# alenxav/bWGR

Measured on AMD Instinct MI355X. Metric: MCMC iter/sec (full marker sweep), higher is better.
Workload: dtype f32 scalars, fixed-point / f64 residual, int8 genotypes; 1 GPU; c4: synthetic n=10000 x p=1000000 int8, BayesB pi=0.99 (1.2% of the markers in the model at the last sweep), exact chain (blocked sweep, block=128, 40 slabs x 256 rows + 1 sequencer, the chain alone on the GPU: 80 streamers x 128 rows, engine generation 3, lag 12 blocks); n=10000, p=1000000, model=BayesB, df=5, chains=1

## Files before the change

### bwgr_amd/csrc/sweep3.hip.h

```cpp
#pragma once
#include "sweep2.hip.h"

namespace bwgr {

#ifdef BWGR_STAMPS
#define S3ST_DECL unsigned long long ph3[8] = {0, 0, 0, 0, 0, 0, 0, 0}, tl3 = __builtin_amdgcn_s_memtime()
#define S3ST(k, cond) do { if ((BWGR_STAMPS == 1 || (BWGR_STAMPS == 2 && ((k) == 0 || (k) == 1 || (k) == 4)) || (BWGR_STAMPS == 3 && ((k) == 0 || (k) == 4) && blockIdx.x == 0 && threadIdx.x == 0) || (BWGR_STAMPS == 4 && (k) <= 5 && blockIdx.x == 0 && threadIdx.x == 0)) && (cond)) { const unsigned long long t_ = __builtin_amdgcn_s_memtime(); ph3[k] += t_ - tl3; tl3 = t_; } } while (0)
#define S3ST_FLUSH(base, cond) do { if ((cond) && a.stamps) for (int k_ = 0; k_ < 8; ++k_) atomicAdd(&a.stamps[(base) + k_], ph3[k_]); } while (0)
#else
#define S3ST_DECL do { } while (0)
#define S3ST(k, cond) do { } while (0)
#define S3ST_FLUSH(base, cond) do { } while (0)
#endif

static constexpr int S3_MAXD = 16;
static constexpr int S3_LSTRIDE = 2 * SW_MAXM + 2;
static constexpr int S3_ND = 7;
static constexpr int S3_RING = S3_MAXD * SW_MAXM;
static constexpr int S3_GPD_BYTES = 16384;
static constexpr int S3_ROWSLOT = 1024;
static constexpr int S3_NRX = 8;
static constexpr int S3_OS = 12;
static constexpr int S3_NFW = 4;
static constexpr int S3_NFL = 8;
// ... 227 lines not shown
  s += (size_t)2 * S3_NFW * S3_NFL * SW_MAXM * (g16 ? 2 : 4);
  if (g16) s += (size_t)3 * S3_GPD_BYTES + (size_t)S3_NRX * S3_ROWSLOT;
  s += (size_t)3 * S3_QRAW_BYTES;
  return s + 256 + 512;
}

__device__ __forceinline__ void s3_streamer(const Sweep3Args &A) {
#ifdef BWGR_EXPERIMENTS
  const int SDBG = A.dbg;
#else
  constexpr int SDBG = 0;
#endif
  extern __shared__ __attribute__((aligned(16))) unsigned char smem[];
  const SweepArgs &a = A.a;
  const int tid = threadIdx.x, lane = tid & 63, wave = tid >> 6;
  const int m16 = lane & 15, grp = lane >> 4;
  const int w = s3_stream_index(A);
  const unsigned long long *lists_w = A.lists;
  const int m = a.m, R = a.R, R3 = A.R3, Rp = R3 + 16, D = A.D;
  const int slab = w / A.sub, hsub = w - slab * A.sub;
  const int nb = a.blk_end - a.blk_begin;
  const int NU = R3 >> 6;
  const int ND = 8 - NU;
  const int cprs = (R3 == 256) ? 4 : (R3 == 128 ? 3 : 2);
  const int8_t *Xs = reinterpret_cast<const int8_t *>(a.X) + (size_t)slab * a.p * R + (size_t)hsub * R3;
  const int64_t row0 = (int64_t)slab * R + (int64_t)hsub * R3;
  uint32_t *abortw = a.xflags + (size_t)a.K * SW_FLAG_STRIDE;
  const size_t tile_b = (size_t)SW_MAXM * Rp;
  int8_t *tile0 = reinterpret_cast<int8_t *>(smem);
  size_t off = 2 * tile_b;
  int8_t *edig0 = reinterpret_cast<int8_t *>(smem + off); off += (size_t)2 * 16 * Rp;
  int8_t *ddig0 = reinterpret_cast<int8_t *>(smem + off); off += (size_t)2 * 16 * S2_DP;
  int *outu = reinterpret_cast<int *>(smem + off); off += (size_t)64 * S3_OS * 4 * 4;
  int *outd = reinterpret_cast<int *>(smem + off); off += (size_t)8 * 32 * S3_OS * 4;
  uint32_t *ctl_s = reinterpret_cast<uint32_t *>(smem + off);
  const int sh = a.sc->e3_sh;
  const double S = s3_pow2(sh), invS = s3_pow2(-sh);
  auto blk_j0 = [&](int b) { return (a.blk_begin + b) * m; };
  auto blk_m = [&](int b) { return min(m, a.p - (a.blk_begin + b) * m); };

  for (int i = tid; i < (int)((2 * 16 * Rp + 2 * 16 * S2_DP) / 4); i += SW_THREADS) reinterpret_cast<uint32_t *>(edig0)[i] = 0u;
  if (tid < 16) ctl_s[tid] = 0u;
  long long e_own = 0;
  const bool upd = wave < NU;
  if (upd) e_own = __double2ll_rn(a.e[row0 + 64 * wave + lane] * S);

  s3_u4 ta0 = {0, 0, 0, 0}, ta1 = ta0, ta2 = ta0, ta3 = ta0, tb0 = ta0, tb1 = ta0, tb2 = ta0, tb3 = ta0;
#define S3_TILE_EACH(X) X(0, tp0) X(1, tp1) X(2, tp2) X(3, tp3)
#define S3_ISSUE1(u, name) { const int cc_ = min(tid + (u) * SW_THREADS, tot_ - 1); const int jj_ = min(cc_ >> cprs, mBt_ - 1), ii_ = cc_ & ((1 << cprs) - 1); \
    name = __builtin_nontemporal_load(reinterpret_cast<const s3_u4 *>(Xs + (size_t)(j0t_ + jj_) * R + ii_ * 16)); }
#define S3_TILE_ISSUE(b_) do { const int j0t_ = blk_j0(b_), mBt_ = blk_m(b_), tot_ = m << cprs; S3_TILE_EACH(S3_ISSUE1) } while (0)
#define S3_COMMIT1(u, name) { const int c_ = tid + (u) * SW_THREADS; if (c_ < tot_) { const int jj_ = c_ >> cprs, ii_ = c_ & ((1 << cprs) - 1); \
    *reinterpret_cast<s3_u4 *>(dst_ + (size_t)jj_ * Rp + ii_ * 16) = name; } }
#define S3_TILE_COMMIT(b_) do { int8_t *dst_ = tile0 + (size_t)((b_) & 1) * tile_b; const int tot_ = m << cprs; S3_TILE_EACH(S3_COMMIT1) } while (0)

  auto fold_list = [&](int bs, unsigned long long pre) -> int {
    const int Bs = a.blk_begin + bs;
    const unsigned long long *L = lists_w + (size_t)Bs * S3_LSTRIDE;
    const int8_t *col = Xs + (size_t)(Bs * m) * R + 64 * wave + lane;
    const uint64_t t0 = wall_clock64();
    unsigned spins = 0;
    unsigned long long hv = __builtin_amdgcn_readfirstlane((uint32_t)pre) | ((unsigned long long)__builtin_amdgcn_readfirstlane((uint32_t)(pre >> 32)) << 32);
    while (!s3_epoch_is(hv, A.epoch)) {
      hv = ld_agent_raw64(L);
      hv = __builtin_amdgcn_readfirstlane((uint32_t)hv) | ((unsigned long long)__builtin_amdgcn_readfirstlane((uint32_t)(hv >> 32)) << 32);
      if (s3_epoch_is(hv, A.epoch)) break;
      if ((++spins & 63u) == 0u) {
// ... 18 lines not shown
        }
        __builtin_amdgcn_s_sleep(1);
      }
      const uint32_t wlo = (uint32_t)wv, whi = (uint32_t)(wv >> 32);
      for (int e0 = 0; e0 < nw / 2; e0 += 8) {
        int xb[8]; long long cq[8];
#pragma unroll
        for (int u = 0; u < 8; ++u) {
          const int ee = min(e0 + u, nw / 2 - 1);
          const uint32_t a0 = __builtin_amdgcn_readlane(wlo, 1 + 2 * ee), a1 = __builtin_amdgcn_readlane(whi, 1 + 2 * ee);
          const uint32_t b0 = __builtin_amdgcn_readlane(wlo, 2 + 2 * ee);
          const int k = (int)(a1 & 0xFFu);
          cq[u] = (e0 + u < nw / 2) ? (long long)(((unsigned long long)b0 << 32) | (unsigned long long)a0) : 0ll;
          xb[u] = upd ? (int)col[(size_t)k * R] : 0;
        }
#pragma unroll
        for (int u = 0; u < 8; ++u) e_own -= (long long)xb[u] * cq[u];
      }
    }
    return 1;
  };

  {
    s3_u4 &tp0 = ta0, &tp1 = ta1, &tp2 = ta2, &tp3 = ta3;
    S3_TILE_ISSUE(0);
    S3_TILE_COMMIT(0);
    if (nb > 2) S3_TILE_ISSUE(2);
  }
  if (nb > 1) { s3_u4 &tp0 = tb0, &tp1 = tb1, &tp2 = tb2, &tp3 = tb3; S3_TILE_ISSUE(1); }
  float drej_pre = a.ps.blocks[a.blk_begin].drej[tid & (SW_MAXM - 1)];
  unsigned long long lpre = 0ull;
  __syncthreads();
  S3ST_DECL;
  const bool st_u = (w == 0 && tid == 0), st_d = (w == 0 && tid == 64 * NU);

  auto step = [&](int b, s3_u4 &tp0, s3_u4 &tp1, s3_u4 &tp2, s3_u4 &tp3) -> bool {
    const int mB = blk_m(b), par = b & 1;
    S3ST(0, st_u || st_d);
    int8_t *tile = tile0 + (size_t)par * tile_b;
    int8_t *edig = edig0 + (size_t)par * 16 * Rp;
    int8_t *ddig = ddig0 + (size_t)par * 16 * S2_DP;
    if (b >= D && upd && !(SDBG & 512)) { if (!fold_list(b - D, lpre)) ctl_s[0] = 1u; }
    S3ST(1, st_u);
    if (upd) {
      if ((unsigned long long)(e_own + (1ll << 54)) >> 55) ctl_s[1] = 1u;
      s3_put_digits7(e_own, edig + 64 * wave + lane, Rp);
    } else if (tid >= SW_THREADS - SW_MAXM) {
      const double qd = (tid - (SW_THREADS - SW_MAXM) < mB) ? rint((double)drej_pre * S) : 0.0;
      if (!(fabs(qd) < 18014398509481984.0)) ctl_s[1] = 1u;
      s3_put_digits7((long long)qd, ddig + (tid - (SW_THREADS - SW_MAXM)), S2_DP);
    }
    S3ST(2, st_u);
#if defined(BWGR_STAMPS) && BWGR_STAMPS == 2
    S3ST(0, st_u || st_d);
    asm volatile("s_waitcnt lgkmcnt(0)\n\ts_barrier" ::: "memory");
    S3ST(4, st_u || st_d);
#else
    asm volatile("s_waitcnt lgkmcnt(0)\n\ts_barrier" ::: "memory");
    S3ST(3, st_u || st_d);
#endif
    if (ctl_s[0]) { if (tid == 0) a.sc->error = 1u; return false; }
    if (b + 1 < nb) S3_TILE_COMMIT(b + 1);
    S3ST(6, st_u || st_d);
    {
      const int bn1 = min(b + 1, nb - 1);
      drej_pre = a.ps.blocks[a.blk_begin + bn1].drej[tid & (SW_MAXM - 1)];
      lpre = ld_agent_raw64(lists_w + (size_t)(a.blk_begin + max(bn1 - D, 0)) * S3_LSTRIDE + lane);
// ... 84 lines not shown
  if (upd && ((unsigned long long)(e_own + (1ll << 54)) >> 55)) ctl_s[1] = 1u;
  __syncthreads();
  if (ctl_s[0]) { if (tid == 0) a.sc->error = 1u; return; }
  if (ctl_s[1] && tid == 0) a.sc->error = 2u;
  if (upd) a.e[row0 + 64 * wave + lane] = (double)e_own * invS;
#undef S3_TILE_EACH
#undef S3_ISSUE1
#undef S3_TILE_ISSUE
#undef S3_COMMIT1
#undef S3_TILE_COMMIT
}

template <int R3, int NTB>
__device__ __forceinline__ void s3_streamer_dma(const Sweep3Args &A) {
#ifdef BWGR_EXPERIMENTS
  const int SDBG = A.dbg;
#else
  constexpr int SDBG = 0;
#endif
  extern __shared__ __attribute__((aligned(16))) unsigned char smem[];
  const SweepArgs &a = A.a;
  const int tid = threadIdx.x, lane = tid & 63, wave = tid >> 6;
  const int m16 = lane & 15, grp = lane >> 4;
  const int w = s3_stream_index(A);
  const unsigned long long *lists_w = A.lists;
  const int m = a.m, R = a.R, D = A.D;
  constexpr int Rp = R3 + 16;
  constexpr int CH = R3 / 16;
  constexpr int MPP = 1024 / R3;
  constexpr int NPC = SW_MAXM / MPP;
  static_assert(R3 == 128 || R3 == 256, "sixteen or thirty-two pieces");
  const int slab = w / A.sub, hsub = w - slab * A.sub;
  const int nb = a.blk_end - a.blk_begin;
  constexpr int NU = R3 >> 6, ND = 8 - NU;
  const int8_t *Xs = reinterpret_cast<const int8_t *>(a.X) + (size_t)slab * a.p * R + (size_t)hsub * R3;
  const int64_t row0 = (int64_t)slab * R + (int64_t)hsub * R3;
  uint32_t *abortw = a.xflags + (size_t)a.K * SW_FLAG_STRIDE;
  constexpr size_t tile_b = (size_t)SW_MAXM * R3;
  int8_t *tile0 = reinterpret_cast<int8_t *>(smem);
  size_t off = NTB * tile_b;
  const uint32_t tile_la = (uint32_t)__builtin_amdgcn_readfirstlane((int)(uint32_t)(uintptr_t)(__attribute__((address_space(3))) const unsigned char *)smem);
  int8_t *edig0 = reinterpret_cast<int8_t *>(smem + off); off += (size_t)2 * 16 * Rp;
  int8_t *ddig0 = reinterpret_cast<int8_t *>(smem + off); off += (size_t)2 * 16 * S2_DP;
  int *outu = reinterpret_cast<int *>(smem + off); off += (size_t)64 * S3_OS * 4 * 4;
  int *outd = reinterpret_cast<int *>(smem + off); off += (size_t)8 * 32 * S3_OS * 4;
  uint32_t *ctl_s = reinterpret_cast<uint32_t *>(smem + off); off += 64;
  float *drej_s = reinterpret_cast<float *>(smem + off);
  const uint32_t drej_la = (uint32_t)__builtin_amdgcn_readfirstlane((int)(uint32_t)(uintptr_t)(__attribute__((address_space(3))) const unsigned char *)drej_s);
  const int sh = a.sc->e3_sh;
  const double S = s3_pow2(sh), invS = s3_pow2(-sh);
  auto blk_j0 = [&](int b) { return (a.blk_begin + b) * m; };
  auto blk_m = [&](int b) { return min(m, a.p - (a.blk_begin + b) * m); };

  for (int i = tid; i < (int)((2 * 16 * Rp + 2 * 16 * S2_DP) / 4); i += SW_THREADS) reinterpret_cast<uint32_t *>(edig0)[i] = 0u;
  if (tid < 16) ctl_s[tid] = 0u;
  long long e_own = 0;
  const bool upd = wave < NU;
  if (upd) e_own = __double2ll_rn(a.e[row0 + 64 * wave + lane] * S);

  static_assert(NU == 2, "waves 0-1 update, 2-5 dots, 6-7 DMA");
  constexpr int NDOT = 4, PPW = NPC / 2;
  constexpr int LPS = PPW + 2;
  const uint32_t lane_mk = (uint32_t)(lane / CH), lane_cr = (uint32_t)(lane % CH);
  const int j_lo = a.blk_begin * m, j_hi = min(a.p, a.blk_end * m);
  const int wvs = __builtin_amdgcn_readfirstlane(wave);
  auto drej_issue = [&](int t) {
    const unsigned char *src = reinterpret_cast<const unsigned char *>(a.ps.blocks[a.blk_begin + max(0, min(t, nb - 1))].drej);
    const uint32_t la = drej_la + (uint32_t)((max(t, 0) % NTB) * SW_MAXM * 4);
    s3_dma4s(src, (uint32_t)lane * 4u, la);
    s3_dma4s(src, 256u + (uint32_t)lane * 4u, la + 256u);
  };
  auto tile_issue = [&](int t) {
    if (wvs < 6) return;
    const int jb = blk_j0(min(t, nb - 1));
    const uint32_t la0 = tile_la + (uint32_t)__builtin_amdgcn_readfirstlane((int)((t % NTB) * (int)tile_b));
#pragma unroll
    for (int u = 0; u < PPW; ++u) {
      const int pc = (wvs - 6) + 2 * u;
      const int jl = MPP * pc + (int)lane_mk;
      const int jj = min(jb + jl, j_hi - 1);
      const uint32_t voff = (uint32_t)(jj - j_lo) * (uint32_t)R + ((lane_cr ^ ((uint32_t)jl & (uint32_t)(CH - 1))) * 16u);
      s3_dma16s(reinterpret_cast<const unsigned char *>(Xs + (size_t)j_lo * R), voff, la0 + (uint32_t)pc * 1024u);
    }
    drej_issue(t + 1);
  };

  auto fold_list = [&](int bs, unsigned long long pre, int e_first = 0) -> int {
    const int Bs = a.blk_begin + bs;
    const unsigned long long *L = lists_w + (size_t)Bs * S3_LSTRIDE;
    const int8_t *col = Xs + (size_t)(Bs * m) * R + 64 * wave + lane;
    const uint64_t t0 = wall_clock64();
    unsigned spins = 0;
    unsigned long long hv = __builtin_amdgcn_readfirstlane((uint32_t)pre) | ((unsigned long long)__builtin_amdgcn_readfirstlane((uint32_t)(pre >> 32)) << 32);
    while (!s3_epoch_is(hv, A.epoch)) {
// ... 56 lines not shown
    const unsigned long long hv = __builtin_amdgcn_readfirstlane((uint32_t)wv) | ((unsigned long long)__builtin_amdgcn_readfirstlane((uint32_t)(wv >> 32)) << 32);
    const int cnt = (int)(uint32_t)hv, nw = min(62, 2 * max(cnt, 0));
    const bool ok = bs >= 0 && s3_epoch_is(hv, A.epoch) && __ballot(lane >= 1 && lane <= nw && !s3_epoch_is(wv, A.epoch)) == 0ull;
    const int8_t *col = Xs + (size_t)((a.blk_begin + max(bs, 0)) * m) * R + 64 * wave + lane;
    const uint32_t wlo = (uint32_t)wv, whi = (uint32_t)(wv >> 32);
    const int ne = ok ? nw / 2 : 0;
#define S3_PRE1(U_, XP_, CP_) { \
      const int ee = min(U_, max(ne - 1, 0)); \
      const uint32_t a0 = __builtin_amdgcn_readlane(wlo, 1 + 2 * ee), a1 = __builtin_amdgcn_readlane(whi, 1 + 2 * ee), b0 = __builtin_amdgcn_readlane(wlo, 2 + 2 * ee); \
      CP_ = (U_ < ne) ? (long long)(((unsigned long long)b0 << 32) | (unsigned long long)a0) : 0ll; \
      XP_ = (int)col[(size_t)(ne > 0 ? (int)(a1 & 0xFFu) : 0) * R]; }
    S3_PRE1(0, xp0, cp0) S3_PRE1(1, xp1, cp1) S3_PRE1(2, xp2, cp2) S3_PRE1(3, xp3, cp3)
#undef S3_PRE1
    np = (bs < 0) ? 0 : (ok ? cnt : -1);
  };
  auto fold_pre = [&](int bs) -> int {
#ifdef BWGR_EXPERIMENTS
    if (w == 0 && tid == 0 && a.stamps && (SDBG & (1 << 21))) { atomicAdd(&a.stamps[203], 1ull); if (np < 0) atomicAdd(&a.stamps[202], 1ull); }
#endif
    if (np < 0) return fold_list(bs, 0ull);
    e_own -= (long long)xp0 * cp0 + (long long)xp1 * cp1 + (long long)xp2 * cp2 + (long long)xp3 * cp3;
    return (np > NPRE) ? fold_list(bs, 0ull, NPRE) : 1;
  };

  if (wvs >= 6) drej_issue(0);
  for (int t = 0; t < NTB - 1; ++t) tile_issue(t);
  if (wvs < NU) {
    lmid = ld_agent_raw64(lists_w + (size_t)(a.blk_begin + max(min(1, nb - 1) - D, 0)) * S3_LSTRIDE + lane);
    if (BWGR_WORDS2) lw1 = ld_agent_raw64(lists_w + (size_t)(a.blk_begin + max(min(2, nb - 1) - D, 0)) * S3_LSTRIDE + lane);
  }
  asm volatile("s_waitcnt vmcnt(0)" ::: "memory");
  __syncthreads();
  S3ST_DECL;
  const bool st_u = (w == 0 && tid == 0), st_d = (w == 0 && tid == 64 * NU);

  constexpr int WN = (NTB - 2) * LPS;
#define S3_DMA_BARRIER() do { if (wvs >= 6) asm volatile("s_waitcnt vmcnt(%0)" : : "n"(WN) : "memory"); asm volatile("s_waitcnt lgkmcnt(0)\n\ts_barrier" ::: "memory"); } while (0)
  auto step = [&](int b, auto par_c) -> bool {
    constexpr int PP = decltype(par_c)::value;
    const int mB = blk_m(b), par = b & 1;
    S3ST(0, st_u || st_d);
    int8_t *tile = tile0 + (size_t)(b % NTB) * tile_b;
    int8_t *edig = edig0 + (size_t)par * 16 * Rp;
    int8_t *ddig = ddig0 + (size_t)par * 16 * S2_DP;
    if (b >= D && upd && !(SDBG & 512)) { if (!fold_pre(b - D)) ctl_s[0] = 1u; }
#ifndef BWGR_FOLD_EARLY
#define BWGR_FOLD_EARLY 1
#endif
    if (BWGR_FOLD_EARLY && wvs < NU) {
      if (!(SDBG & 512)) fold_prefetch((b + 1 < nb) ? b + 1 - D : -1, par_c);
      S3_PAR(lmid, lw1) = ld_agent_raw64(lists_w + (size_t)(a.blk_begin + max(min(b + 2 + BWGR_WORDS2, nb - 1) - D, 0)) * S3_LSTRIDE + lane);
    }
    S3ST(1, st_u);
    if (upd) {
      if ((unsigned long long)(e_own + (1ll << 54)) >> 55) ctl_s[1] = 1u;
      s3_put_digits7(e_own, edig + 64 * wave + lane, Rp);
    } else if (tid >= SW_THREADS - SW_MAXM) {
      const double qd = (tid - (SW_THREADS - SW_MAXM) < mB) ? rint((double)drej_s[(b % NTB) * SW_MAXM + (tid - (SW_THREADS - SW_MAXM))] * S) : 0.0;
      if (!(fabs(qd) < 18014398509481984.0)) ctl_s[1] = 1u;
      s3_put_digits7((long long)qd, ddig + (tid - (SW_THREADS - SW_MAXM)), S2_DP);
    }
    S3ST(2, st_u);
#if defined(BWGR_STAMPS) && BWGR_STAMPS == 2
    S3ST(0, st_u || st_d);
    S3_DMA_BARRIER();
    S3ST(4, st_u || st_d);
#else
    S3_DMA_BARRIER();
    S3ST(3, st_u || st_d);
#endif
    if (ctl_s[0]) { if (tid == 0) a.sc->error = 1u; return false; }
    tile_issue(b + NTB - 1);
    S3ST(6, st_u || st_d);
    {
      if (!BWGR_FOLD_EARLY && wvs < NU) {
        if (!(SDBG & 512)) fold_prefetch((b + 1 < nb) ? b + 1 - D : -1, par_c);
        S3_PAR(lmid, lw1) = ld_agent_raw64(lists_w + (size_t)(a.blk_begin + max(min(b + 2 + BWGR_WORDS2, nb - 1) - D, 0)) * S3_LSTRIDE + lane);
      }
    }
    S3ST(7, st_u || st_d);
    S3ST(4, st_u || st_d);
    if (upd) {
      s2_v4i acc0 = {0, 0, 0, 0}, acc1 = acc0, acc2 = acc0, acc3 = acc0;
      const uint32_t tile_lds = tile_la + (uint32_t)((b % NTB) * (int)tile_b);
      const uint32_t q8 = (uint32_t)((lane & 15) >> 1), p8 = (uint32_t)(lane & 1);
      const uint32_t cw = (uint32_t)(4 * wave);
      for (int s0 = 0; s0 < ((SDBG & 256) ? 0 : mB); s0 += 64) {
        const uint32_t rowA = tile_lds + (uint32_t)(s0 + 16 * grp + (int)q8) * (uint32_t)R3 + 8u * p8;
        const uint32_t a0 = rowA + ((((cw + 0u) ^ q8) & (uint32_t)(CH - 1)) << 4), a1 = rowA + ((((cw + 1u) ^ q8) & (uint32_t)(CH - 1)) << 4);
        const uint32_t a2 = rowA + ((((cw + 2u) ^ q8) & (uint32_t)(CH - 1)) << 4), a3 = rowA + ((((cw + 3u) ^ q8) & (uint32_t)(CH - 1)) << 4);
        typedef int s3_v2i __attribute__((ext_vector_type(2)));
        s3_v2i x0, x1, x2, x3, y0, y1, y2, y3;
        asm volatile("ds_read_b64_tr_b8 %0, %8\n\tds_read_b64_tr_b8 %4, %8 offset:1024\n\t"
                     "ds_read_b64_tr_b8 %1, %9\n\tds_read_b64_tr_b8 %5, %9 offset:1024\n\t"
                     "ds_read_b64_tr_b8 %2, %10\n\tds_read_b64_tr_b8 %6, %10 offset:1024\n\t"
                     "ds_read_b64_tr_b8 %3, %11\n\tds_read_b64_tr_b8 %7, %11 offset:1024\n\ts_waitcnt lgkmcnt(0)"
                     : "=&v"(x0), "=&v"(x1), "=&v"(x2), "=&v"(x3), "=&v"(y0), "=&v"(y1), "=&v"(y2), "=&v"(y3)
                     : "v"(a0), "v"(a1), "v"(a2), "v"(a3) : "memory");
        static_assert(R3 == 128, "offset:1024 = eight markers of 128 bytes");
        const s2_v4i bv = *reinterpret_cast<const s2_v4i *>(ddig + (size_t)m16 * S2_DP + s0 + 16 * grp);
        acc0 = __builtin_amdgcn_mfma_i32_16x16x64_i8(s2_v4i{x0[0], x0[1], y0[0], y0[1]}, bv, acc0, 0, 0, 0);
        acc1 = __builtin_amdgcn_mfma_i32_16x16x64_i8(s2_v4i{x1[0], x1[1], y1[0], y1[1]}, bv, acc1, 0, 0, 0);
        acc2 = __builtin_amdgcn_mfma_i32_16x16x64_i8(s2_v4i{x2[0], x2[1], y2[0], y2[1]}, bv, acc2, 0, 0, 0);
        acc3 = __builtin_amdgcn_mfma_i32_16x16x64_i8(s2_v4i{x3[0], x3[1], y3[0], y3[1]}, bv, acc3, 0, 0, 0);
      }
      int *ou = outu + (size_t)wave * 64 * S3_OS;
      if (m16 < 8) {
        int *op = ou + (size_t)(4 * grp) * S3_OS + m16;
#pragma unroll
        for (int reg = 0; reg < 4; ++reg) {
          op[(reg + 0) * S3_OS] = acc0[reg]; op[(reg + 16) * S3_OS] = acc1[reg];
          op[(reg + 32) * S3_OS] = acc2[reg]; op[(reg + 48) * S3_OS] = acc3[reg];
        }
      }
      asm volatile("s_waitcnt lgkmcnt(0)" ::: "memory");
      {
        const int4 o0 = *reinterpret_cast<const int4 *>(ou + (size_t)lane * S3_OS);
        const int4 o1 = *reinterpret_cast<const int4 *>(ou + (size_t)lane * S3_OS + 4);
        long long v = (long long)o0.x + ((long long)o0.y << 8) + ((long long)o0.z << 16) + ((long long)o0.w << 24);
        v += ((long long)o1.x << 32) + ((long long)o1.y << 40) + ((long long)o1.z << 48);
        e_own -= v;
      }
      S3ST(5, st_u);
    } else {
      for (int gm = wave - NU; wvs < NU + NDOT && 16 * gm < m; gm += 2 * NDOT) {
        const int gm2 = gm + NDOT;
        const bool two = 16 * gm2 < m;
        const int8_t *bp = edig + (size_t)m16 * Rp + 16 * grp;
        const int8_t *ap = tile + (size_t)(16 * gm + m16) * R3;
        const int8_t *ap2 = tile + (size_t)(16 * (two ? gm2 : gm) + m16) * R3;
        s2_v4i acc = {0, 0, 0, 0}, acc2 = acc;
        for (int r = 0; r < ((SDBG & 256) ? 0 : R3); r += 64) {
          const s2_v4i bv = *reinterpret_cast<const s2_v4i *>(bp + r);
          const int so = (((grp + (r >> 4)) ^ (m16 & (CH - 1))) << 4);
          acc = __builtin_amdgcn_mfma_i32_16x16x64_i8(bv, *reinterpret_cast<const s2_v4i *>(ap + so), acc, 0, 0, 0);
          acc2 = __builtin_amdgcn_mfma_i32_16x16x64_i8(bv, *reinterpret_cast<const s2_v4i *>(ap2 + so), acc2, 0, 0, 0);
        }
        if (grp < 2) {
          const long long w1 = (long long)acc[0] + ((long long)acc[1] << 8) + ((long long)acc[2] << 16) + ((long long)acc[3] << 24);
          const long long w2 = (long long)acc2[0] + ((long long)acc2[1] << 8) + ((long long)acc2[2] << 16) + ((long long)acc2[3] << 24);
          unsigned long long *qs = A.qsum + ((size_t)(a.blk_begin + b) * SW_MAXM + 16 * gm + m16) * 2 + grp;
          if (!(SDBG & 8)) {
            __hip_atomic_fetch_add((gu64_t *)qs, (unsigned long long)((w1 << 8) + 1), __ATOMIC_RELAXED, __HIP_MEMORY_SCOPE_AGENT);
            if (two) __hip_atomic_fetch_add((gu64_t *)(qs + (size_t)(16 * (gm2 - gm)) * 2), (unsigned long long)((w2 << 8) + 1), __ATOMIC_RELAXED, __HIP_MEMORY_SCOPE_AGENT);
          }
        }
      }
      S3ST(5, st_d);
    }
    return true;
  };
  for (int b = 0; b < nb; b += 2) {
    if (!step(b, std::integral_constant<int, 0>{})) return;
    if (b + 1 < nb && !step(b + 1, std::integral_constant<int, 1>{})) return;
  }
  asm volatile("s_waitcnt vmcnt(0)" ::: "memory");
#undef S3_DMA_BARRIER
#undef S3_PAR
  S3ST_FLUSH(0, st_u); S3ST_FLUSH(8, st_d);
  if (upd && !(SDBG & 512)) for (int bs = max(0, nb - D); bs < nb; ++bs) {
    if (!fold_list(bs, 0ull)) { ctl_s[0] = 1u; break; }
  }
  if (upd && ((unsigned long long)(e_own + (1ll << 54)) >> 55)) ctl_s[1] = 1u;
  __syncthreads();
  if (ctl_s[0]) { if (tid == 0) a.sc->error = 1u; return; }
  if (ctl_s[1] && tid == 0) a.sc->error = 2u;
  if (upd) a.e[row0 + 64 * wave + lane] = (double)e_own * invS;
}

template <typename GT, bool CEN = false>
__device__ __forceinline__ void s3_sequencer(const Sweep3Args &A) {
#ifdef BWGR_EXPERIMENTS
  const int SDBG = A.dbg;
#else
  constexpr int SDBG = 0;
#endif
  extern __shared__ __attribute__((aligned(16))) unsigned char smem[];
  const SweepArgs &a = A.a;
  const int tid = threadIdx.x, lane = tid & 63, wave = tid >> 6;
  const int m = a.m, nb = a.blk_end - a.blk_begin, D = A.D, pstride = a.pstride;
  size_t off = 0;
  StageBuf *stage = reinterpret_cast<StageBuf *>(smem + off); off += 3 * sizeof(StageBuf);
  double *spec_s = reinterpret_cast<double *>(smem + off); off += (size_t)3 * 2 * SW_MAXM * sizeof(double);
  double *q_s = reinterpret_cast<double *>(smem + off); off += (size_t)2 * SW_MAXM * sizeof(double);
  double *far_s = reinterpret_cast<double *>(smem + off); off += (size_t)2 * S3_NFW * SW_MAXM * sizeof(double);
  float *state_s = reinterpret_cast<float *>(smem + off); off += (size_t)2 * 3 * SW_MAXM * sizeof(float);
  double *accC = reinterpret_cast<double *>(smem + off); off += (size_t)S3_RING * sizeof(double);
  float2 *accS = reinterpret_cast<float2 *>(smem + off); off += (size_t)S3_RING * sizeof(float2);
// ... 229 lines not shown
      const int t = lane + 64 * h;
      if (t < mBc) {
        const float bn = sp[t], dn = sp[SW_MAXM + t];
        a.b[j0c + t] = bn;
        a.d[j0c + t] = dn;
        if (vbv) a.vb[j0c + t] = (float)((double)(Sb + bn * bn) / (h ? ch1 : ch0));
        sum_d += (double)dn;
        sum_b2 = fma((double)bn, (double)bn, sum_b2);
      }
    }
    const int p0 = pos_s[c & 31], cnt = (pos_s[(c + 1) & 31] - p0) & (ring - 1);
    unsigned long long *L = A.lists + (size_t)blk * S3_LSTRIDE;
    for (int w0 = 0; w0 < 1 + 2 * cnt; w0 += 64) {
      const int wi = w0 + lane;
      if (wi < 1 + 2 * cnt) {
        unsigned long long v;
        if (wi == 0) v = s3_hdr(A.epoch, cnt);
        else {
          const int sl = (p0 + ((wi - 1) >> 1)) & (ring - 1);
          const float2 st2 = accS[sl];
          const long long cq = (long long)rint((double)st2.x * S) - (long long)rint((double)st2.y * S);
          v = ((wi - 1) & 1) ? (((unsigned long long)A.epoch << 40) | (0xEEull << 32) | ((unsigned long long)cq >> 32))
                             : (((unsigned long long)A.epoch << 40) | ((unsigned long long)(uint32_t)(accK[sl] & 0xFF) << 32) | ((unsigned long long)cq & 0xFFFFFFFFull));
        }
        st_agent_raw64(L + wi, v);
      }
    }
  };
#ifndef BWGR_ROLEBAR
#define BWGR_ROLEBAR 1
#endif
#define S3_ROLE_BARRIER() do { if (BWGR_ROLEBAR) asm volatile("s_waitcnt lgkmcnt(0)\n\ts_barrier" ::: "memory"); } while (0)
  const int wvu = __builtin_amdgcn_readfirstlane(wave);
  auto helper_phase = [&](int c) {
    if (wvu == 1) { if (!(SDBG & 32768)) { if (!poll_q(c)) ctrl_s[0] = 0; } S3ST(2, tid == 64); S3_ROLE_BARRIER(); }
    else if (wvu <= 3) { if (!(SDBG & 8192)) {
      const int o_p0 = f_p0, o_cnt = f_cnt, o_n = f_n; const double o_cf = f_cf;
      far_plan_a(c + 1);
      stage_issue(c + 1, 0);
      far_plan_b(c + 1, wave);
      stage_issue(c + 1, 1);
      far_plan_c(c + 1);
      stage_issue(c + 1, 2);
      S3_STG_WAIT();
      far_consume(c, wave, o_p0, o_cnt, o_n, o_cf);
      far_request(c + 1, wave);
    } S3ST(2, tid == 128 || tid == 192); S3_ROLE_BARRIER(); }
    else if (wvu == 4) { far_touch(c); S3_ROLE_BARRIER(); }
    else if (wvu <= 6) {
      const int o_p0 = f_p0, o_cnt = f_cnt, o_n = f_n; const double o_cf = f_cf;
      far_plan(c + 1, wave - 5);
      asm volatile("s_waitcnt vmcnt(0) lgkmcnt(0)" ::: "memory");
      S3ST(5, tid == 320);
      far_consume(c, wave - 5, o_p0, o_cnt, o_n, o_cf);
      S3ST(6, tid == 320);
      far_request(c + 1, wave - 5);
      S3ST(7, tid == 320);
      S3ST(2, tid == 384);
      S3_ROLE_BARRIER();
    }
    else { if (c >= 2 && !(SDBG & 4096)) finish_block(c - 2); touch(c + PF); S3ST(2, tid == 448); S3_ROLE_BARRIER(); }
  };

  if (tid < 40) ctrl_s[tid] = (tid == 0) ? 1 : 0;
  if (tid >= 64 && tid < 64 + S3_MAXD) gx_s[tid - 64] = reinterpret_cast<const unsigned char *>(A.gx[tid - 64]);
  __syncthreads();
  if (wave == 1) { poll_request(0); poll_request(1); if (!poll_q(0)) ctrl_s[0] = 0; }
  else if (wave == 2 || wave == 3) { stage_issue(0); stage_issue(1); S3_STG_WAIT(); far_consume(0, wave, 0, 0, 0, 0.0); far_plan(1, wave); far_request(1, wave); }
  else if (wave >= 5 && wave <= 6) { far_consume(0, wave - 5, 0, 0, 0, 0.0); far_plan(1, wave - 5); far_request(1, wave - 5); }
  else if (wave == 7) { for (int c = 0; c < PF; ++c) touch(c); if ((a.flags & SWF_VB_VEC) && !A.skip_vb) chi_request(0); }
  __syncthreads();
  if (ctrl_s[0] == 0) { if (tid == 0) a.sc->error = 1u; asm volatile("s_waitcnt vmcnt(0)" ::: "memory"); return; }

  const bool sq0 = (tid == 0), sq1 = (tid == 64), sq2 = (tid == 128), sq4 = (tid == 320), sq3 = (tid == 192), sq6 = (tid == 384), sq7 = (tid == 448);
  const int tabp0 = 2 * (lane * (m - 1) - lane * (lane - 1) / 2 - lane - 1);
  const int tabp1 = 2 * ((64 + lane) * (m - 1) - (64 + lane) * (63 + lane) / 2 - (64 + lane) - 1);
  const uint32_t rolane = (uint32_t)min(lane * 4, rowbytes - 4);
  const uint32_t rolane16 = (uint32_t)min(lane * 16, 2 * rowbytes - 16);
  constexpr bool near12 = G16;
  const unsigned char *gpd_lane = gpd_s + 2 * lane;
  int gpd_off = 0;
  const uint32_t rowx_la = (uint32_t)__builtin_amdgcn_readfirstlane((int)(uint32_t)(uintptr_t)(__attribute__((address_space(3))) const unsigned char *)rowx_s);
  const bool altb2 = (a.flags & SWF_ALT_B2) != 0;
  if (wave == 0 && !(SDBG & 1)) __builtin_amdgcn_s_setprio(3);
  double rnext0 = 0.0, rnext1 = 0.0, rnxt20 = 0.0, rnxt21 = 0.0;
  int pend_n = 0, pend_p = 0;
  bool pend_u1 = false, pend_u2 = false;
  const double ninv = a.ninv;
  const double cen_u0 = CEN ? a.sc->cen_u0 : 0.0;
  double cenU = cen_u0;
  const GT *gx0_w0 = reinterpret_cast<const GT *>(A.gx[0]) + (size_t)a.blk_begin * m * m, *gx1_w0 = reinterpret_cast<const GT *>(A.gx[1]) + (size_t)a.blk_begin * m * m;
  const unsigned char *g12_w0 = A.gx12 + (size_t)a.blk_begin * m * 2 * rowbytes;
  for (int b = 0; b < nb; ++b) {
    const int mB = blk_m(b), blk = a.blk_begin + b;
    const bool have_next = (b + 1 < nb);
    S3ST(0, sq0 || sq1 || sq2 || sq4 || sq3 || sq6 || sq7);
    if (wvu == 0 && !(SDBG & 16384)) {
      const StageBuf &st = stage[b % 3];
      const double *sps = spec_s + (size_t)(b % 3) * 2 * SW_MAXM;
      const double *qd = q_s + (size_t)(b & 1) * SW_MAXM;
      const double *fd = far_s + (size_t)(b & 1) * S3_NFW * SW_MAXM;
      const int pos0 = pos_s[b & 31];
      const GT *gp = gp_all + (size_t)blk * pstride;
      const bool use1 = have_next && D >= 2;
      const GT *g1 = (G16 || use1) ? gx0_w0 + (size_t)(b + 1) * (uint32_t)(m * m) : gp;
      const bool use2 = (b + 2 < nb) && D >= 3;
      const GT *g2 = (G16 || use2) ? gx1_w0 + (size_t)(b + 2) * (uint32_t)(m * m) : gp;
      const unsigned char *g12b = g12_w0 + (size_t)b * (uint32_t)(m * 2 * rowbytes);
      const int l0 = lane, l1 = 64 + lane;
      const int l1c = min(l1, m - 1), l0c = min(l0, m - 1);
      const float b0a = st.b0[l0], b0b = st.b0[l1], b2a = st.b2[l0], b2b = st.b2[l1], dra = st.drej[l0], drb = st.drej[l1];
      const float taa = st.tacc[l0], tab = st.tacc[l1], tra = st.trej[l0], trb = st.trej[l1];
      const double xba = (double)st.xxb0[l0], xbb = (double)st.xxb0[l1];
      const double rda = st.rden[l0], rdb = st.rden[l1], sza = st.sdz1[l0], szb = st.sdz1[l1];
      double gja = sps[SW_MAXM + l0], gjb = sps[SW_MAXM + l1];
      double r0 = (qd[l0] - sps[l0]) - ((fd[l0] + fd[SW_MAXM + l0]) + (fd[2 * SW_MAXM + l0] + fd[3 * SW_MAXM + l0]));
      double r1 = (qd[l1] - sps[l1]) - ((fd[l1] + fd[SW_MAXM + l1]) + (fd[2 * SW_MAXM + l1] + fd[3 * SW_MAXM + l1]));
      if constexpr (G16) {
        if (pend_n > 0) {
          asm volatile("s_waitcnt vmcnt(0) lgkmcnt(0)" ::: "memory");
          for (int i_ = 0; i_ < pend_n; ++i_) {
            const double cf_ = accC[(pend_p + i_) & (ring - 1)];
            const uint16_t *rw1_ = reinterpret_cast<const uint16_t *>(rowx_s + (size_t)i_ * S3_ROWSLOT);
            const uint16_t *rw2_ = rw1_ + m;
            const uint32_t x1a_ = rw1_[l0c], x1b_ = rw1_[l1c], x2a_ = rw2_[l0c], x2b_ = rw2_[l1c];
            const double c1_ = pend_u1 ? cf_ : 0.0, c2_ = pend_u2 ? cf_ : 0.0;
            rnext0 = fma(-(double)x1a_, c1_, rnext0); rnext1 = fma(-(double)x1b_, c1_, rnext1);
            rnxt20 = fma(-(double)x2a_, c2_, rnxt20); rnxt21 = fma(-(double)x2b_, c2_, rnxt21);
          }
          pend_n = 0;
// ... 95 lines not shown
        }
      }
      if (mB > 64 && (!(SDBG & 128))) {
        const int cnt1 = mB - 64;
        unsigned long long live1 = (cnt1 >= 64) ? ~0ull : ((1ull << cnt1) - 1ull);
        for (;;) {
          float d1f; unsigned long long acc;
          S3_EVAL(r1, xbb, rdb, szb, b0b, D2b, D2sb, gjb, tab, trb, 64, d1f, acc)
          const unsigned long long bal = acc & live1;
          if (bal == 0ull) break;
          const int js = (int)__builtin_ctzll(bal);
          live1 &= (~1ull << js);
          am1 |= 1ull << js;
          S3_INCLUDE(64, d1f, drb)
        }
      }
#undef S3_EVAL
#undef S3_INCLUDE
      S3ST(5, sq0);
      if constexpr (G16) { pend_n = nslot; pend_p = pos0 + napp; pend_u1 = use1; pend_u2 = use2; }
#undef S3_APPLY_ROWS
      S3ST(2, sq0);
      {
        float *sp = state_s + (size_t)(b & 1) * 2 * SW_MAXM;
        const float b1a = (float)fma(r0 + xba, rda, sza), b1b = (float)fma(r1 + xbb, rdb, szb);
        const bool ia = ((am0 >> lane) & 1ull) != 0ull, ib = ((am1 >> lane) & 1ull) != 0ull;
        sp[l0] = ia ? b1a : b2a; sp[l1] = ib ? b1b : b2b;
        sp[SW_MAXM + l0] = ia ? 1.0f : 0.0f; sp[SW_MAXM + l1] = ib ? 1.0f : 0.0f;
      }
      if (lane == 0) pos_s[(b + 1) & 31] = (pos0 + nacc) & (ring - 1);
      S3ST(3, sq0);
      gpd_off = (gpd_off == 2 * S3_GPD_BYTES) ? 0 : gpd_off + S3_GPD_BYTES;
      S3_ROLE_BARRIER();
    } else if (have_next && wvu != 0) {
      helper_phase(b + 1);
      S3ST(1, sq1 || sq2 || sq4 || sq3 || sq6 || sq7);
    } else S3_ROLE_BARRIER();
    if (!BWGR_ROLEBAR) asm volatile("s_waitcnt lgkmcnt(0)\n\ts_barrier" ::: "memory");
    S3ST(4, sq0 || sq1 || sq2 || sq4 || sq3 || sq6 || sq7);
    if (ctrl_s[0] == 0) { if (tid == 0) a.sc->error = 1u; asm volatile("s_waitcnt vmcnt(0)" ::: "memory"); return; }
  }
  S3ST_FLUSH(16, sq0); S3ST_FLUSH(24, sq1); S3ST_FLUSH(32, sq2); S3ST_FLUSH(40, sq4); S3ST_FLUSH(48, sq3); S3ST_FLUSH(56, sq6); S3ST_FLUSH(64, sq7);
  if constexpr (CEN) { if (tid == 0) a.sc->cen_c = cenU - cen_u0; }
  if (wave >= 1 && wave <= 4) asm volatile("s_waitcnt vmcnt(0)" ::: "memory");
  if (wave == 7) {
    if (nb >= 2) finish_block(nb - 2);
    finish_block(nb - 1);
#pragma unroll
    for (int o = 32; o > 0; o >>= 1) { sum_d += __shfl_down(sum_d, o, 64); sum_b2 += __shfl_down(sum_b2, o, 64); }
    if (lane == 0) { a.sc->sum_d += sum_d; a.sc->sum_b2 += sum_b2; }
  }
}

template <typename GT, bool ROWS>
__device__ __forceinline__ void s3_prefetcher(const Sweep3Args &A) {
  const SweepArgs &a = A.a;
  const int tid = threadIdx.x, nb = a.blk_end - a.blk_begin;
  constexpr int AHEAD = 16, NPB = 4;
  uint32_t *abortw = a.xflags + (size_t)a.K * SW_FLAG_STRIDE;
  const size_t gpbytes = (size_t)a.pstride * sizeof(GT);
  uint32_t sink = 0u;
  const size_t o = (size_t)tid * 128;
  for (int c0 = 0; c0 < nb; c0 += NPB) {
    const int clast = min(c0 + NPB, nb) - 1;
    if (clast >= AHEAD) {
      const unsigned long long *L = A.lists + (size_t)(a.blk_begin + clast - AHEAD) * S3_LSTRIDE;
      const uint64_t t0 = wall_clock64();
      unsigned spins = 0;
      for (;;) {
        if (s3_epoch_is(ld_agent_raw64(L), A.epoch)) break;
        if ((++spins & 63u) == 0u && (ld_agent_u32(abortw) != 0u || wall_clock64() - t0 > SW_TIMEOUT_TICKS)) return;
        __builtin_amdgcn_s_sleep(4);
      }
    }
    uint32_t v[NPB][3];
    const size_t g12bytes = (size_t)a.m * 2 * a.m * sizeof(GT);
#pragma unroll
    for (int u = 0; u < NPB; ++u) {
      const int blk = a.blk_begin + min(c0 + u, nb - 1);
      if (ROWS) {
        v[u][0] = *reinterpret_cast<const uint32_t *>(A.gx12 + (size_t)blk * g12bytes + min(o, g12bytes - 4));
        v[u][1] = 0u; v[u][2] = 0u;
      } else {
        const unsigned char *gpb = reinterpret_cast<const unsigned char *>(A.gp) + (size_t)blk * gpbytes;
// ... 28 lines not shown
```

Before: 95.11 iter/s.

## Specialise streamer and sequencer loops per wave role at compile time

The streamer step loop is templated on the wave role (update, dot, DMA), so each wave runs a loop with its role fixed at compile time and only DMA waves issue tile loads. The sequencer's per-block loop is split into separate loops for each wave role, with wave 0's large block body kept in its own branch. The goal is to remove per-iteration role branching and to lower register pressure, since each role's live state no longer has to share one loop body. The cost is larger code size, plus the risk that barrier counts diverge between roles if any loop exits differently.

```diff
diff --git a/bwgr_amd/csrc/sweep3.hip.h b/bwgr_amd/csrc/sweep3.hip.h
--- a/bwgr_amd/csrc/sweep3.hip.h
+++ b/bwgr_amd/csrc/sweep3.hip.h
@@ -283,7 +283,7 @@
   int8_t *edig0 = reinterpret_cast<int8_t *>(smem + off); off += (size_t)2 * 16 * Rp;
   int8_t *ddig0 = reinterpret_cast<int8_t *>(smem + off); off += (size_t)2 * 16 * S2_DP;
   int *outu = reinterpret_cast<int *>(smem + off); off += (size_t)64 * S3_OS * 4 * 4;
-  int *outd = reinterpret_cast<int *>(smem + off); off += (size_t)8 * 32 * S3_OS * 4;
+  off += (size_t)8 * 32 * S3_OS * 4;
   uint32_t *ctl_s = reinterpret_cast<uint32_t *>(smem + off);
   const int sh = a.sc->e3_sh;
   const double S = s3_pow2(sh), invS = s3_pow2(-sh);
@@ -368,7 +368,7 @@
   unsigned long long lpre = 0ull;
   __syncthreads();
   S3ST_DECL;
-  const bool st_u = (w == 0 && tid == 0), st_d = (w == 0 && tid == 64 * NU);
+  [[maybe_unused]] const bool st_u = (w == 0 && tid == 0), st_d = (w == 0 && tid == 64 * NU);
 
   auto step = [&](int b, s3_u4 &tp0, s3_u4 &tp1, s3_u4 &tp2, s3_u4 &tp3) -> bool {
     const int mB = blk_m(b), par = b & 1;
@@ -519,7 +519,7 @@
   static_assert(R3 == 128 || R3 == 256, "sixteen or thirty-two pieces");
   const int slab = w / A.sub, hsub = w - slab * A.sub;
   const int nb = a.blk_end - a.blk_begin;
-  constexpr int NU = R3 >> 6, ND = 8 - NU;
+  constexpr int NU = R3 >> 6;
   const int8_t *Xs = reinterpret_cast<const int8_t *>(a.X) + (size_t)slab * a.p * R + (size_t)hsub * R3;
   const int64_t row0 = (int64_t)slab * R + (int64_t)hsub * R3;
   uint32_t *abortw = a.xflags + (size_t)a.K * SW_FLAG_STRIDE;
@@ -530,7 +530,7 @@
   int8_t *edig0 = reinterpret_cast<int8_t *>(smem + off); off += (size_t)2 * 16 * Rp;
   int8_t *ddig0 = reinterpret_cast<int8_t *>(smem + off); off += (size_t)2 * 16 * S2_DP;
   int *outu = reinterpret_cast<int *>(smem + off); off += (size_t)64 * S3_OS * 4 * 4;
-  int *outd = reinterpret_cast<int *>(smem + off); off += (size_t)8 * 32 * S3_OS * 4;
+  off += (size_t)8 * 32 * S3_OS * 4;
   uint32_t *ctl_s = reinterpret_cast<uint32_t *>(smem + off); off += 64;
   float *drej_s = reinterpret_cast<float *>(smem + off);
   const uint32_t drej_la = (uint32_t)__builtin_amdgcn_readfirstlane((int)(uint32_t)(uintptr_t)(__attribute__((address_space(3))) const unsigned char *)drej_s);
@@ -547,6 +547,7 @@
 
   static_assert(NU == 2, "waves 0-1 update, 2-5 dots, 6-7 DMA");
   constexpr int NDOT = 4, PPW = NPC / 2;
+  static_assert(NU + NDOT == 6 && SW_THREADS - SW_MAXM == 64 * (NU + NDOT), "the DMA waves (role 2) are the last two: they digitise the rejected steps");
   constexpr int LPS = PPW + 2;
   const uint32_t lane_mk = (uint32_t)(lane / CH), lane_cr = (uint32_t)(lane % CH);
   const int j_lo = a.blk_begin * m, j_hi = min(a.p, a.blk_end * m);
@@ -669,30 +670,32 @@
   asm volatile("s_waitcnt vmcnt(0)" ::: "memory");
   __syncthreads();
   S3ST_DECL;
-  const bool st_u = (w == 0 && tid == 0), st_d = (w == 0 && tid == 64 * NU);
+  [[maybe_unused]] const bool st_u = (w == 0 && tid == 0), st_d = (w == 0 && tid == 64 * NU);
 
   constexpr int WN = (NTB - 2) * LPS;
-#define S3_DMA_BARRIER() do { if (wvs >= 6) asm volatile("s_waitcnt vmcnt(%0)" : : "n"(WN) : "memory"); asm volatile("s_waitcnt lgkmcnt(0)\n\ts_barrier" ::: "memory"); } while (0)
-  auto step = [&](int b, auto par_c) -> bool {
+#define S3_DMA_BARRIER() do { if constexpr (DMA) asm volatile("s_waitcnt vmcnt(%0)" : : "n"(WN) : "memory"); asm volatile("s_waitcnt lgkmcnt(0)\n\ts_barrier" ::: "memory"); } while (0)
+  auto step = [&](int b, auto par_c, auto role_c) -> bool {
     constexpr int PP = decltype(par_c)::value;
+    constexpr int RL = decltype(role_c)::value;
+    constexpr bool UPD = RL == 0, DMA = RL == 2;
     const int mB = blk_m(b), par = b & 1;
     S3ST(0, st_u || st_d);
     int8_t *tile = tile0 + (size_t)(b % NTB) * tile_b;
     int8_t *edig = edig0 + (size_t)par * 16 * Rp;
     int8_t *ddig = ddig0 + (size_t)par * 16 * S2_DP;
-    if (b >= D && upd && !(SDBG & 512)) { if (!fold_pre(b - D)) ctl_s[0] = 1u; }
+    if (b >= D && UPD && !(SDBG & 512)) { if (!fold_pre(b - D)) ctl_s[0] = 1u; }
 #ifndef BWGR_FOLD_EARLY
 #define BWGR_FOLD_EARLY 1
 #endif
-    if (BWGR_FOLD_EARLY && wvs < NU) {
+    if (BWGR_FOLD_EARLY && UPD) {
       if (!(SDBG & 512)) fold_prefetch((b + 1 < nb) ? b + 1 - D : -1, par_c);
       S3_PAR(lmid, lw1) = ld_agent_raw64(lists_w + (size_t)(a.blk_begin + max(min(b + 2 + BWGR_WORDS2, nb - 1) - D, 0)) * S3_LSTRIDE + lane);
     }
     S3ST(1, st_u);
-    if (upd) {
+    if constexpr (UPD) {
       if ((unsigned long long)(e_own + (1ll << 54)) >> 55) ctl_s[1] = 1u;
       s3_put_digits7(e_own, edig + 64 * wave + lane, Rp);
-    } else if (tid >= SW_THREADS - SW_MAXM) {
+    } else if constexpr (DMA) {
       const double qd = (tid - (SW_THREADS - SW_MAXM) < mB) ? rint((double)drej_s[(b % NTB) * SW_MAXM + (tid - (SW_THREADS - SW_MAXM))] * S) : 0.0;
       if (!(fabs(qd) < 18014398509481984.0)) ctl_s[1] = 1u;
       s3_put_digits7((long long)qd, ddig + (tid - (SW_THREADS - SW_MAXM)), S2_DP);
@@ -707,17 +710,17 @@
     S3ST(3, st_u || st_d);
 #endif
     if (ctl_s[0]) { if (tid == 0) a.sc->error = 1u; return false; }
-    tile_issue(b + NTB - 1);
+    if constexpr (DMA) tile_issue(b + NTB - 1);
     S3ST(6, st_u || st_d);
     {
-      if (!BWGR_FOLD_EARLY && wvs < NU) {
+      if (!BWGR_FOLD_EARLY && UPD) {
         if (!(SDBG & 512)) fold_prefetch((b + 1 < nb) ? b + 1 - D : -1, par_c);
         S3_PAR(lmid, lw1) = ld_agent_raw64(lists_w + (size_t)(a.blk_begin + max(min(b + 2 + BWGR_WORDS2, nb - 1) - D, 0)) * S3_LSTRIDE + lane);
       }
     }
     S3ST(7, st_u || st_d);
     S3ST(4, st_u || st_d);
-    if (upd) {
+    if constexpr (UPD) {
       s2_v4i acc0 = {0, 0, 0, 0}, acc1 = acc0, acc2 = acc0, acc3 = acc0;
       const uint32_t tile_lds = tile_la + (uint32_t)((b % NTB) * (int)tile_b);
       const uint32_t q8 = (uint32_t)((lane & 15) >> 1), p8 = (uint32_t)(lane & 1);
@@ -759,8 +762,8 @@
         e_own -= v;
       }
       S3ST(5, st_u);
-    } else {
-      for (int gm = wave - NU; wvs < NU + NDOT && 16 * gm < m; gm += 2 * NDOT) {
+    } else if constexpr (RL == 1) {
+      for (int gm = wave - NU; 16 * gm < m; gm += 2 * NDOT) {
         const int gm2 = gm + NDOT;
         const bool two = 16 * gm2 < m;
         const int8_t *bp = edig + (size_t)m16 * Rp + 16 * grp;
@@ -787,10 +790,18 @@
     }
     return true;
   };
-  for (int b = 0; b < nb; b += 2) {
-    if (!step(b, std::integral_constant<int, 0>{})) return;
-    if (b + 1 < nb && !step(b + 1, std::integral_constant<int, 1>{})) return;
-  }
+  auto run = [&](auto role_c) -> bool {
+    for (int b = 0; b < nb; b += 2) {
+      if (!step(b, std::integral_constant<int, 0>{}, role_c)) return false;
+      if (b + 1 < nb && !step(b + 1, std::integral_constant<int, 1>{}, role_c)) return false;
+    }
+    return true;
+  };
+  bool ok;
+  if (wvs < NU) ok = run(std::integral_constant<int, 0>{});
+  else if (wvs < NU + NDOT) ok = run(std::integral_constant<int, 1>{});
+  else ok = run(std::integral_constant<int, 2>{});
+  if (!ok) return;
   asm volatile("s_waitcnt vmcnt(0)" ::: "memory");
 #undef S3_DMA_BARRIER
 #undef S3_PAR
@@ -1086,35 +1097,6 @@
 #endif
 #define S3_ROLE_BARRIER() do { if (BWGR_ROLEBAR) asm volatile("s_waitcnt lgkmcnt(0)\n\ts_barrier" ::: "memory"); } while (0)
   const int wvu = __builtin_amdgcn_readfirstlane(wave);
-  auto helper_phase = [&](int c) {
-    if (wvu == 1) { if (!(SDBG & 32768)) { if (!poll_q(c)) ctrl_s[0] = 0; } S3ST(2, tid == 64); S3_ROLE_BARRIER(); }
-    else if (wvu <= 3) { if (!(SDBG & 8192)) {
-      const int o_p0 = f_p0, o_cnt = f_cnt, o_n = f_n; const double o_cf = f_cf;
-      far_plan_a(c + 1);
-      stage_issue(c + 1, 0);
-      far_plan_b(c + 1, wave);
-      stage_issue(c + 1, 1);
-      far_plan_c(c + 1);
-      stage_issue(c + 1, 2);
-      S3_STG_WAIT();
-      far_consume(c, wave, o_p0, o_cnt, o_n, o_cf);
-      far_request(c + 1, wave);
-    } S3ST(2, tid == 128 || tid == 192); S3_ROLE_BARRIER(); }
-    else if (wvu == 4) { far_touch(c); S3_ROLE_BARRIER(); }
-    else if (wvu <= 6) {
-      const int o_p0 = f_p0, o_cnt = f_cnt, o_n = f_n; const double o_cf = f_cf;
-      far_plan(c + 1, wave - 5);
-      asm volatile("s_waitcnt vmcnt(0) lgkmcnt(0)" ::: "memory");
-      S3ST(5, tid == 320);
-      far_consume(c, wave - 5, o_p0, o_cnt, o_n, o_cf);
-      S3ST(6, tid == 320);
-      far_request(c + 1, wave - 5);
-      S3ST(7, tid == 320);
-      S3ST(2, tid == 384);
-      S3_ROLE_BARRIER();
-    }
-    else { if (c >= 2 && !(SDBG & 4096)) finish_block(c - 2); touch(c + PF); S3ST(2, tid == 448); S3_ROLE_BARRIER(); }
-  };
 
   if (tid < 40) ctrl_s[tid] = (tid == 0) ? 1 : 0;
   if (tid >= 64 && tid < 64 + S3_MAXD) gx_s[tid - 64] = reinterpret_cast<const unsigned char *>(A.gx[tid - 64]);
@@ -1125,31 +1107,41 @@
   else if (wave == 7) { for (int c = 0; c < PF; ++c) touch(c); if ((a.flags & SWF_VB_VEC) && !A.skip_vb) chi_request(0); }
   __syncthreads();
   if (ctrl_s[0] == 0) { if (tid == 0) a.sc->error = 1u; asm volatile("s_waitcnt vmcnt(0)" ::: "memory"); return; }
-
-  const bool sq0 = (tid == 0), sq1 = (tid == 64), sq2 = (tid == 128), sq4 = (tid == 320), sq3 = (tid == 192), sq6 = (tid == 384), sq7 = (tid == 448);
-  const int tabp0 = 2 * (lane * (m - 1) - lane * (lane - 1) / 2 - lane - 1);
-  const int tabp1 = 2 * ((64 + lane) * (m - 1) - (64 + lane) * (63 + lane) / 2 - (64 + lane) - 1);
-  const uint32_t rolane = (uint32_t)min(lane * 4, rowbytes - 4);
-  const uint32_t rolane16 = (uint32_t)min(lane * 16, 2 * rowbytes - 16);
-  constexpr bool near12 = G16;
-  const unsigned char *gpd_lane = gpd_s + 2 * lane;
-  int gpd_off = 0;
-  const uint32_t rowx_la = (uint32_t)__builtin_amdgcn_readfirstlane((int)(uint32_t)(uintptr_t)(__attribute__((address_space(3))) const unsigned char *)rowx_s);
-  const bool altb2 = (a.flags & SWF_ALT_B2) != 0;
-  if (wave == 0 && !(SDBG & 1)) __builtin_amdgcn_s_setprio(3);
-  double rnext0 = 0.0, rnext1 = 0.0, rnxt20 = 0.0, rnxt21 = 0.0;
-  int pend_n = 0, pend_p = 0;
-  bool pend_u1 = false, pend_u2 = false;
-  const double ninv = a.ninv;
-  const double cen_u0 = CEN ? a.sc->cen_u0 : 0.0;
-  double cenU = cen_u0;
-  const GT *gx0_w0 = reinterpret_cast<const GT *>(A.gx[0]) + (size_t)a.blk_begin * m * m, *gx1_w0 = reinterpret_cast<const GT *>(A.gx[1]) + (size_t)a.blk_begin * m * m;
-  const unsigned char *g12_w0 = A.gx12 + (size_t)a.blk_begin * m * 2 * rowbytes;
-  for (int b = 0; b < nb; ++b) {
-    const int mB = blk_m(b), blk = a.blk_begin + b;
-    const bool have_next = (b + 1 < nb);
-    S3ST(0, sq0 || sq1 || sq2 || sq4 || sq3 || sq6 || sq7);
-    if (wvu == 0 && !(SDBG & 16384)) {
+  [[maybe_unused]] const bool sq0 = (tid == 0), sq1 = (tid == 64), sq2 = (tid == 128), sq4 = (tid == 320), sq3 = (tid == 192), sq6 = (tid == 384), sq7 = (tid == 448);
+#define S3_BLOCK_END(SQ_, ABORT_) \
+    if (!BWGR_ROLEBAR) asm volatile("s_waitcnt lgkmcnt(0)\n\ts_barrier" ::: "memory"); \
+    S3ST(4, SQ_); \
+    if (ctrl_s[0] == 0) { asm volatile("s_waitcnt vmcnt(0)" ::: "memory"); ABORT_; }
+  auto helper_loop = [&](auto &&phase, const bool sq) -> bool {
+    for (int b = 0; b < nb; ++b) {
+      S3ST(0, sq);
+      if (b + 1 < nb) { phase(b + 1); S3ST(1, sq); }
+      else S3_ROLE_BARRIER();
+      S3_BLOCK_END(sq, return false)
+    }
+    return true;
+  };
+  if (wvu == 0) {
+    const int tabp0 = 2 * (lane * (m - 1) - lane * (lane - 1) / 2 - lane - 1);
+    const int tabp1 = 2 * ((64 + lane) * (m - 1) - (64 + lane) * (63 + lane) / 2 - (64 + lane) - 1);
+    const uint32_t rolane16 = (uint32_t)min(lane * 16, 2 * rowbytes - 16);
+    const unsigned char *gpd_lane = gpd_s + 2 * lane;
+    int gpd_off = 0;
+    const uint32_t rowx_la = (uint32_t)__builtin_amdgcn_readfirstlane((int)(uint32_t)(uintptr_t)(__attribute__((address_space(3))) const unsigned char *)rowx_s);
+    const bool altb2 = (a.flags & SWF_ALT_B2) != 0;
+    if (wave == 0 && !(SDBG & 1)) __builtin_amdgcn_s_setprio(3);
+    double rnext0 = 0.0, rnext1 = 0.0, rnxt20 = 0.0, rnxt21 = 0.0;
+    int pend_n = 0, pend_p = 0;
+    bool pend_u1 = false, pend_u2 = false;
+    const double ninv = a.ninv;
+    const double cen_u0 = CEN ? a.sc->cen_u0 : 0.0;
+    double cenU = cen_u0;
+    const GT *gx0_w0 = reinterpret_cast<const GT *>(A.gx[0]) + (size_t)a.blk_begin * m * m, *gx1_w0 = reinterpret_cast<const GT *>(A.gx[1]) + (size_t)a.blk_begin * m * m;
+    const unsigned char *g12_w0 = A.gx12 + (size_t)a.blk_begin * m * 2 * rowbytes;
+    if (!(SDBG & 1)) __builtin_amdgcn_s_setprio(3);
+    auto block = [&](int b) {
+      const int mB = blk_m(b), blk = a.blk_begin + b;
+      const bool have_next = (b + 1 < nb);
       const StageBuf &st = stage[b % 3];
       const double *sps = spec_s + (size_t)(b % 3) * 2 * SW_MAXM;
       const double *qd = q_s + (size_t)(b & 1) * SW_MAXM;
@@ -1311,24 +1303,62 @@
       S3ST(3, sq0);
       gpd_off = (gpd_off == 2 * S3_GPD_BYTES) ? 0 : gpd_off + S3_GPD_BYTES;
       S3_ROLE_BARRIER();
-    } else if (have_next && wvu != 0) {
-      helper_phase(b + 1);
-      S3ST(1, sq1 || sq2 || sq4 || sq3 || sq6 || sq7);
-    } else S3_ROLE_BARRIER();
-    if (!BWGR_ROLEBAR) asm volatile("s_waitcnt lgkmcnt(0)\n\ts_barrier" ::: "memory");
-    S3ST(4, sq0 || sq1 || sq2 || sq4 || sq3 || sq6 || sq7);
-    if (ctrl_s[0] == 0) { if (tid == 0) a.sc->error = 1u; asm volatile("s_waitcnt vmcnt(0)" ::: "memory"); return; }
-  }
-  S3ST_FLUSH(16, sq0); S3ST_FLUSH(24, sq1); S3ST_FLUSH(32, sq2); S3ST_FLUSH(40, sq4); S3ST_FLUSH(48, sq3); S3ST_FLUSH(56, sq6); S3ST_FLUSH(64, sq7);
-  if constexpr (CEN) { if (tid == 0) a.sc->cen_c = cenU - cen_u0; }
-  if (wave >= 1 && wave <= 4) asm volatile("s_waitcnt vmcnt(0)" ::: "memory");
-  if (wave == 7) {
+    };
+    for (int b = 0; b < nb; ++b) {
+      S3ST(0, sq0);
+      if (!(SDBG & 16384)) block(b);
+      else S3_ROLE_BARRIER();
+      S3_BLOCK_END(sq0, if (tid == 0) a.sc->error = 1u; return)
+    }
+    S3ST_FLUSH(16, sq0);
+    if constexpr (CEN) { if (tid == 0) a.sc->cen_c = cenU - cen_u0; }
+  } else if (wvu == 1) {
+    if (!helper_loop([&](int c) { if (!(SDBG & 32768)) { if (!poll_q(c)) ctrl_s[0] = 0; } S3ST(2, tid == 64); S3_ROLE_BARRIER(); }, sq1)) return;
+    S3ST_FLUSH(24, sq1);
+    asm volatile("s_waitcnt vmcnt(0)" ::: "memory");
+  } else if (wvu <= 3) {
+    if (!helper_loop([&](int c) {
+      if (!(SDBG & 8192)) {
+        const int o_p0 = f_p0, o_cnt = f_cnt, o_n = f_n; const double o_cf = f_cf;
+        far_plan_a(c + 1);
+        stage_issue(c + 1, 0);
+        far_plan_b(c + 1, wave);
+        stage_issue(c + 1, 1);
+        far_plan_c(c + 1);
+        stage_issue(c + 1, 2);
+        S3_STG_WAIT();
+        far_consume(c, wave, o_p0, o_cnt, o_n, o_cf);
+        far_request(c + 1, wave);
+      }
+      S3ST(2, tid == 128 || tid == 192); S3_ROLE_BARRIER(); }, sq2 || sq3)) return;
+    S3ST_FLUSH(32, sq2); S3ST_FLUSH(48, sq3);
+    asm volatile("s_waitcnt vmcnt(0)" ::: "memory");
+  } else if (wvu == 4) {
+    if (!helper_loop([&](int c) { far_touch(c); S3_ROLE_BARRIER(); }, false)) return;
+    asm volatile("s_waitcnt vmcnt(0)" ::: "memory");
+  } else if (wvu <= 6) {
+    if (!helper_loop([&](int c) {
+      const int o_p0 = f_p0, o_cnt = f_cnt, o_n = f_n; const double o_cf = f_cf;
+      far_plan(c + 1, wave - 5);
+      asm volatile("s_waitcnt vmcnt(0) lgkmcnt(0)" ::: "memory");
+      S3ST(5, tid == 320);
+      far_consume(c, wave - 5, o_p0, o_cnt, o_n, o_cf);
+      S3ST(6, tid == 320);
+      far_request(c + 1, wave - 5);
+      S3ST(7, tid == 320);
+      S3ST(2, tid == 384);
+      S3_ROLE_BARRIER(); }, sq4 || sq6)) return;
+    S3ST_FLUSH(40, sq4); S3ST_FLUSH(56, sq6);
+  } else {
+    if (!helper_loop([&](int c) { if (c >= 2 && !(SDBG & 4096)) finish_block(c - 2); touch(c + PF); S3ST(2, tid == 448); S3_ROLE_BARRIER(); }, sq7)) return;
+    S3ST_FLUSH(64, sq7);
     if (nb >= 2) finish_block(nb - 2);
     finish_block(nb - 1);
 #pragma unroll
     for (int o = 32; o > 0; o >>= 1) { sum_d += __shfl_down(sum_d, o, 64); sum_b2 += __shfl_down(sum_b2, o, 64); }
     if (lane == 0) { a.sc->sum_d += sum_d; a.sc->sum_b2 += sum_b2; }
   }
+#undef S3_BLOCK_END
 }
 
 template <typename GT, bool ROWS>
```

After: 100.3 iter/s, median of 6. 1.05x the previous value.
